# spool-labs/clay

Hardware: AMD Instinct MI355X
Metric: device-resident encode GiB/s at (k=10,m=4,d=13); % of HBM roofline (higher is better)
Workload: dtype u8; 1 GPU; (k=10,m=4,d=13) encode, one 1 GiB stripe per GPU; stripe_input_bytes=1073741824, padded_stripe_bytes=1073745920, chunk_bytes=107374592, sub_chunk_bytes=419432, alpha=256, parallelism=stripe-per-gpu x1

## Files before the change

bench_tools/stream_probe.hip:

```cpp
#include <hip/hip_runtime.h>

#include <algorithm>
#include <cstdlib>
#include <cstdio>
#include <vector>

#include "../clay_amd/csrc/stream_encode.hpp"

using namespace clay::bs;

template <int L, int PROBE>
static float run(BsArgs a, int reps) {
    using Kn = StreamEnc<10, L>;
    (void)hipFuncSetAttribute(reinterpret_cast<const void *>(&k_stream_encode<10, L, PROBE>),
                              hipFuncAttributeMaxDynamicSharedMemorySize, Kn::LDS_BYTES);
    hipEvent_t e0, e1;
    (void)hipEventCreate(&e0);
    (void)hipEventCreate(&e1);
    std::vector<float> t;
    for (int r = 0; r < reps; r++) {
        (void)hipEventRecord(e0);
        k_stream_encode<10, L, PROBE><<<dim3(a.nslots * 8), dim3(Kn::BLOCK), Kn::LDS_BYTES>>>(a);
        (void)hipEventRecord(e1);
        (void)hipEventSynchronize(e1);
        float ms;
        (void)hipEventElapsedTime(&ms, e0, e1);
        if (r >= 3) t.push_back(ms);
    }
    std::sort(t.begin(), t.end());
    return t[t.size() / 2];
}

template <int L, int PROBE, int MAP = 0>
static float run_b2b(BsArgs a, int n, int warm = 50) {
    using Kn = StreamEnc<10, L>;
    (void)hipFuncSetAttribute(reinterpret_cast<const void *>(&k_stream_encode<10, L, PROBE, MAP>),
                              hipFuncAttributeMaxDynamicSharedMemorySize, Kn::LDS_BYTES);
    hipEvent_t e0, e1;
    (void)hipEventCreate(&e0);
    (void)hipEventCreate(&e1);
    for (int i = 0; i < warm; i++)
        k_stream_encode<10, L, PROBE, MAP><<<dim3(a.nslots * 8), dim3(Kn::BLOCK), Kn::LDS_BYTES>>>(a);
    (void)hipEventRecord(e0);
    for (int i = 0; i < n; i++)
        k_stream_encode<10, L, PROBE, MAP><<<dim3(a.nslots * 8), dim3(Kn::BLOCK), Kn::LDS_BYTES>>>(a);
    (void)hipEventRecord(e1);
    (void)hipEventSynchronize(e1);
    float ms;
    (void)hipEventElapsedTime(&ms, e0, e1);
    const hipError_t err = hipGetLastError();
    if (err != hipSuccess) {
        printf("HIP error (probe %d): %s\n", PROBE, hipGetErrorString(err));
        exit(3);
    }
    return ms / float(n);
}

template <int TP, int MAP = 0>
static void timing_report(BsArgs a, int n) {
    using Kn = StreamEnc<10, 4>;
    const int grid = int(a.nslots) * 8;
    const size_t rec = size_t(grid) * 12 * 24;
    uint64_t *tb;
    (void)hipMalloc(&tb, rec * 8);
    (void)hipMemset(tb, 0, rec * 8);
    a.par[4] = reinterpret_cast<uint8_t *>(tb);
    const float ms_plain = run_b2b<4, 0, MAP>(a, n);
    const float ms_tm = run_b2b<4, TP, MAP>(a, n);
    std::vector<uint64_t> h(rec);
    (void)hipMemcpy(h.data(), tb, rec * 8, hipMemcpyDeviceToHost);
    printf("b2b ms: plain %.4f  timing-probe %.4f (s_memtime counts per XCD; cycles below are per tile)\n", ms_plain, ms_tm);
    printf("wave  role     total   bar/vm y0   y1    y2 | math/bar y0   y1    y2 | issue y0  y1    y2 | end g0  g1    g2    g3\n");
    for (int w = 0; w < 12; w++) {
        double v[3][3] = {}, ge[4] = {}, tot = 0;
        int cnt = 0;
        for (int b = 0; b < grid; b++) {
            const uint64_t *p = &h[(size_t(b) * 12 + w) * 24];
            const double nt = double(p[16]);
            if (nt == 0) continue;
            cnt++;
            for (int i = 0; i < 3; i++)
                for (int j = 0; j < 3; j++) v[i][j] += double(p[i * 3 + j]) / nt;
            for (int g = 0; g < 4; g++) ge[g] += double(p[9 + g]) / nt;
            tot += double(p[15] - p[13]) / nt;
        }
        const double G = cnt ? cnt : 1;
        printf("%4d  %-7s %7.0f  %6.0f %6.0f %6.0f | %6.0f %6.0f %6.0f | %6.0f %6.0f %6.0f | %5.0f %5.0f %5.0f %5.0f\n", w,
               w < 8 ? "compute" : "loader", tot / G, v[0][0] / G, v[0][1] / G, v[0][2] / G, v[1][0] / G, v[1][1] / G,
               v[1][2] / G, v[2][0] / G, v[2][1] / G, v[2][2] / G, ge[0] / G, ge[1] / G, ge[2] / G, ge[3] / G);
    }
    fflush(stdout);
    (void)hipFree(tb);
    (void)Kn::BLOCK;
}

int main(int argc, char **argv) {
    const uint32_t sc = argc > 1 ? uint32_t(atoi(argv[1])) : 419432;
    const bool quick = argc > 2;
    const size_t chunk = size_t(sc) * 256;
    uint8_t *data, *par;
    if (hipMalloc(&data, 10 * chunk) != hipSuccess || hipMalloc(&par, 4 * chunk) != hipSuccess) return 1;
    {
        std::vector<uint8_t> h(10 * chunk);
        uint64_t x = 0x9E3779B97F4A7C15ull;
        for (auto &b : h) { x ^= x << 13; x ^= x >> 7; x ^= x << 17; b = uint8_t(x >> 24); }
        (void)hipMemcpy(data, h.data(), h.size(), hipMemcpyHostToDevice);
    }
    BsArgs a{};
    for (int i = 0; i < 10; i++) a.data[i] = data + i * chunk;
    for (int x = 0; x < 4; x++) a.par[x] = par + x * chunk;
    a.sc = sc;
    const uint32_t ralign = argc > 3 ? uint32_t(atoi(argv[3])) : 32u;
    a.tiles_per_xcd = uint32_t(((sc + 7) / 8 + ralign - 1) / ralign * ralign);
    a.nslots = 32;
    const double bytes = 14.0 * chunk;
    auto rep = [&](const char *n, float ms) {
        printf("%-34s %8.4f ms  %7.1f GB/s (algorithmic)\n", n, ms, bytes / (ms * 1e-3) / 1e9);
        fflush(stdout);
    };
    (void)hipFuncSetAttribute(reinterpret_cast<const void *>(&k_stream_encode<10, 2, 0>),
                              hipFuncAttributeMaxDynamicSharedMemorySize, StreamEnc<10, 2>::LDS_BYTES);
    for (int i = 0; i < 300; i++) k_stream_encode<10, 2, 0><<<dim3(a.nslots * 8), dim3(StreamEnc<10, 2>::BLOCK), StreamEnc<10, 2>::LDS_BYTES>>>(a);
    {
        const hipError_t e = hipDeviceSynchronize();
        const hipError_t e2 = hipGetLastError();
        if (e != hipSuccess || e2 != hipSuccess) {
            printf("HIP error after warm-up: %s / %s\n", hipGetErrorString(e), hipGetErrorString(e2));
            return 3;
        }
    }
    if (argc > 2 && argv[2][0] == 't') {
        printf("sc %u segment timing\n", sc);
        timing_report<4096>(a, 200);
        printf("---- deferred end of group (PROBE 8192)\n");
        timing_report<4096 | 8192>(a, 200);
        return 0;
    }
    if (argc > 2 && argv[2][0] == 'd') {
        printf("sc %u deferred end-of-group A/B, back-to-back\n", sc);
        for (int rr = 0; rr < 3; rr++) {
            rep("b2b full", run_b2b<4, 0>(a, 200));
            rep("b2b full, end of group after the next barrier", run_b2b<4, 8192>(a, 200));
            rep("b2b memory only", run_b2b<4, 1>(a, 200));
            rep("b2b memory only, deferred", run_b2b<4, 8193>(a, 200));
            rep("b2b full, no sched barrier between nodes", run_b2b<4, 16384>(a, 200));
            rep("b2b full, sched barrier every 2 nodes", run_b2b<4, 32768>(a, 200));
            rep("b2b full, deferred + every 2 nodes", run_b2b<4, 32768 | 8192>(a, 200));
        }
        return 0;
    }
    if (argc > 2 && argv[2][0] == 'p') {
        printf("sc %u balanced priority A/B, back-to-back\n", sc);
        for (int rr = 0; rr < 3; rr++) {
            rep("b2b full", run_b2b<4, 0>(a, 200));
            rep("b2b full, balanced priority", run_b2b<4, 131072>(a, 200));
            rep("b2b math + stores (no DMA)", run_b2b<4, 2>(a, 200));
            rep("b2b math + stores (no DMA), balanced priority", run_b2b<4, 2 | 131072>(a, 200));
        }
        timing_report<4096 | 131072>(a, 200);
        return 0;
    }
    if (argc > 2 && argv[2][0] == 'v') {
        printf("sc %u variants, back-to-back (200 launches after 50 untimed)\n", sc);
        for (int rr = 0; rr < 3; rr++) {
            rep("b2b full", run_b2b<4, 0>(a, 200));
            rep("b2b memory only (DMA + stores, no math)", run_b2b<4, 1>(a, 200));
            rep("b2b reads only", run_b2b<4, 5>(a, 200));
            rep("b2b stores only", run_b2b<4, 3>(a, 200));
            rep("b2b live reads + math (no stores)", run_b2b<4, 262144>(a, 200));
            rep("b2b live math only (no DMA, no stores)", run_b2b<4, 262146>(a, 200));
            rep("b2b math + stores (no DMA)", run_b2b<4, 2>(a, 200));
            rep("b2b math + stores, no DMA, no barriers", run_b2b<4, 2 | 65536>(a, 200));
            rep("b2b live math only, no barriers", run_b2b<4, 262146 | 65536>(a, 200));
        }
        return 0;
    }
    if (argc > 2 && argv[2][0] == 'n') {
        printf("sc %u lane map A/B, back-to-back (200 launches after 50 untimed)\n", sc);
        if (argv[2][1] == 't') {
            timing_report<4096, 0>(a, 200);
            printf("---- map 3\n");
            timing_report<4096, 3>(a, 200);
            return 0;
        }
        const size_t pbytes = 4 * chunk;
        std::vector<uint8_t> ref(pbytes), got(pbytes);
        auto snap = [&](std::vector<uint8_t> &v) {
            (void)hipDeviceSynchronize();
            (void)hipMemcpy(v.data(), par, pbytes, hipMemcpyDeviceToHost);
        };
        (void)hipMemset(par, 0, pbytes);
        run_b2b<4, 0, 0>(a, 1, 0);
        snap(ref);
        auto check = [&](const char *name) {
            snap(got);
            printf("  bytes %s == map 0: %s\n", name, ref == got ? "yes" : "NO");
            (void)hipMemset(par, 0, pbytes);
        };
        run_b2b<4, 0, 1>(a, 1, 0); check("map 1");
        run_b2b<4, 0, 3>(a, 1, 0); check("map 3");
        run_b2b<4, 0, 4>(a, 1, 0); check("map 4");
        run_b2b<4, 0, 5>(a, 1, 0); check("map 5");
        run_b2b<4, 0, 6>(a, 1, 0); check("map 6");
        run_b2b<4, 0, 7>(a, 1, 0); check("map 7");
        run_b2b<4, 0, 8>(a, 1, 0); check("map 8");
        run_b2b<4, 0, 9>(a, 1, 0); check("map 9");
        if (argv[2][1] == '8') {
            for (int rr = 0; rr < 3; rr++) {
                rep("b2b full, map 0 (round 5)", run_b2b<4, 0, 0>(a, 200));
                rep("b2b full, map 8", run_b2b<4, 0, 8>(a, 200));
                rep("b2b full, map 9 (map 8 without red skip)", run_b2b<4, 0, 9>(a, 200));
                rep("b2b full, map 8, waves 4-7 prio 1", run_b2b<4, 16, 8>(a, 200));
                rep("b2b full, map 8, no sched barriers", run_b2b<4, 16384, 8>(a, 200));
                rep("b2b full, map 8, sched barrier / 2 nodes", run_b2b<4, 32768, 8>(a, 200));
                rep("b2b memory only, map 8", run_b2b<4, 1, 8>(a, 200));
                rep("b2b live math only, map 8", run_b2b<4, 262146, 8>(a, 200));
                rep("b2b live reads + math, map 8", run_b2b<4, 262144, 8>(a, 200));
                rep("b2b math + stores, map 8", run_b2b<4, 2, 8>(a, 200));
            }
            timing_report<4096, 8>(a, 200);
            return 0;
        }
        for (int rr = 0; rr < 3; rr++) {
            rep("b2b full, map 0 (round 5)", run_b2b<4, 0, 0>(a, 200));
            rep("b2b memory only, map 0", run_b2b<4, 1, 0>(a, 200));
            rep("b2b full, map 1 (k 2,3,4 pair 16)", run_b2b<4, 0, 1>(a, 200));
            rep("b2b memory only, map 1", run_b2b<4, 1, 1>(a, 200));
            rep("b2b full, map 3 (map 1, permlane pair 32)", run_b2b<4, 0, 3>(a, 200));
            rep("b2b full, map 4 (k 3,2,4 pair 32)", run_b2b<4, 0, 4>(a, 200));
            rep("b2b memory only, map 4", run_b2b<4, 1, 4>(a, 200));
            rep("b2b full, map 5 (k 4,3,2 pair 64)", run_b2b<4, 0, 5>(a, 200));
            rep("b2b memory only, map 5", run_b2b<4, 1, 5>(a, 200));
            rep("b2b full, map 6 (k 5,4,3 pair 128)", run_b2b<4, 0, 6>(a, 200));
            rep("b2b memory only, map 6", run_b2b<4, 1, 6>(a, 200));
            rep("b2b full, map 7 (k 2,5,4 pair 16)", run_b2b<4, 0, 7>(a, 200));
            rep("b2b memory only, map 7", run_b2b<4, 1, 7>(a, 200));
            rep("b2b full, map 8 (k 4,5,3 pair 64)", run_b2b<4, 0, 8>(a, 200));
            rep("b2b memory only, map 8", run_b2b<4, 1, 8>(a, 200));
            rep("b2b live math only, map 1", run_b2b<4, 262146, 1>(a, 200));
        }
        return 0;
    }
    if (argc > 2 && argv[2][0] == 'w') {
        rep("full", run_b2b<4, 0>(a, 10, 2));
        rep("memory only", run_b2b<4, 1>(a, 10, 2));
        rep("reads only", run_b2b<4, 5>(a, 10, 2));
        rep("stores only", run_b2b<4, 3>(a, 10, 2));
        rep("live reads + math", run_b2b<4, 262144>(a, 10, 2));
        rep("live math only", run_b2b<4, 262146>(a, 10, 2));
        rep("math + stores", run_b2b<4, 2>(a, 10, 2));
        return 0;
    }
    if (argc > 2 && argv[2][0] == 'f') {
        unsigned int *flag;
        (void)hipMalloc(&flag, 4);
        (void)hipMemset(flag, 0, 4);
        a.par[5] = reinterpret_cast<uint8_t *>(flag);
        printf("sc %u no-barrier timing probe (PROBE 4096|65536|2) with bounds checks (524288)\n", sc);
        timing_report<4096 | 65536 | 2 | 524288>(a, 50);
        unsigned int h = 0;
        (void)hipMemcpy(&h, flag, 4, hipMemcpyDeviceToHost);
        printf("bounds flags 0x%x (bits 0-3 parity store of node X, 4-7 ragged store, 8 compute record, 9 loader record)\n", h);
        return 0;
    }
    if (argc > 2 && argv[2][0] == 'a') {
        printf("sc %u (row start mod 128 varies: %s), XCD region %u (alignment %u)\n", sc,
               sc % 128 ? "yes" : "no, rows 128-aligned", a.tiles_per_xcd, ralign);
        for (int rr = 0; rr < 2; rr++) {
            rep("b2b full", run_b2b<4, 0>(a, 200));
            rep("b2b memory only (DMA + stores)", run_b2b<4, 1>(a, 200));
            rep("b2b stores only", run_b2b<4, 3>(a, 200));
            rep("b2b reads only", run_b2b<4, 5>(a, 200));
        }
        return 0;
    }
    if (argc > 2 && argv[2][0] == 'l') {
        printf("sc %u back-to-back loader sweep\n", sc);
        for (int rr = 0; rr < 3; rr++) {
            rep("b2b L4 full", run_b2b<4, 0>(a, 200));
            rep("b2b L2 full", run_b2b<2, 0>(a, 200));
            rep("b2b L1 full", run_b2b<1, 0>(a, 200));
            rep("b2b L4 full, loaders prio 0", run_b2b<4, 8>(a, 200));
        }
        return 0;
    }
    if (argc > 2 && argv[2][0] == 'b') {
        printf("sc %u back-to-back (200 launches after 50 untimed)\n", sc);
        for (int rr = 0; rr < 3; rr++) {
            rep("b2b L4 full (CSE)", run_b2b<4, 0>(a, 200));
            rep("b2b L4 full, no CSE", run_b2b<4, 1024>(a, 200));
            rep("b2b L4 memory only", run_b2b<4, 1>(a, 200));
            rep("b2b L4 math + stores (CSE)", run_b2b<4, 2>(a, 200));
        }
        return 0;
    }
    if (argc > 2 && argv[2][0] == 'm') {
        printf("sc %u tile map (XCD-blocked vs chip round robin), back-to-back\n", sc);
        for (int rr = 0; rr < 3; rr++) {
            rep("b2b full, XCD-blocked", run_b2b<4, 0>(a, 200));
            rep("b2b full, chip RR", run_b2b<4, 2048>(a, 200));
            rep("b2b memory only, XCD-blocked", run_b2b<4, 1>(a, 200));
            rep("b2b memory only, chip RR", run_b2b<4, 2049>(a, 200));
            rep("b2b stores only, XCD-blocked", run_b2b<4, 3>(a, 200));
            rep("b2b stores only, chip RR", run_b2b<4, 2051>(a, 200));
            rep("b2b reads only, XCD-blocked", run_b2b<4, 5>(a, 200));
            rep("b2b reads only, chip RR", run_b2b<4, 2053>(a, 200));
        }
        return 0;
    }
    if (argc > 2 && argv[2][0] == 'x') {
        printf("sc %u cse folds\n", sc);
        for (int rr = 0; rr < 3; rr++) {
            rep("L4 full, row-by-row folds", run<4, 1024>(a, 15));
            rep("L4 full (CSE folds)", run<4, 0>(a, 15));
            rep("L0 full, row-by-row folds", run<0, 1024>(a, 15));
            rep("L0 full (CSE folds)", run<0, 0>(a, 15));
            rep("L4 math + stores, row-by-row folds", run<4, 1026>(a, 15));
            rep("L4 math + stores (CSE folds)", run<4, 2>(a, 15));
        }
        return 0;
    }
    if (argc > 2 && argv[2][0] == 'c') {
        printf("sc %u cache policies\n", sc);
        for (int rr = 0; rr < 2; rr++) {
            rep("L4 full", run<4, 0>(a, 15));
            rep("L4 full, nt loads", run<4, 64>(a, 15));
            rep("L4 full, nt stores", run<4, 256>(a, 15));
            rep("L4 full, nt loads + stores", run<4, 320>(a, 15));
            rep("L4 full, sc1 loads", run<4, 128>(a, 15));
            rep("L4 full, sc1 stores", run<4, 512>(a, 15));
            rep("L4 memory only", run<4, 1>(a, 15));
            rep("L4 memory only, nt loads", run<4, 65>(a, 15));
            rep("L4 memory only, nt stores", run<4, 257>(a, 15));
            rep("L4 memory only, nt both", run<4, 321>(a, 15));
            rep("L4 reads, nt", run<4, 69>(a, 15));
            rep("L4 stores only, nt", run<4, 259>(a, 15));
        }
        return 0;
    }
    if (quick) {
        printf("sc %u\n", sc);
        for (int rr = 0; rr < 2; rr++) {
            rep("L4 full", run<4, 0>(a, 15));
            rep("L4 no math (memory only)", run<4, 1>(a, 15));
            rep("L4 reads", run<4, 5>(a, 15));
            rep("L4 stores only", run<4, 3>(a, 15));
            rep("L4 memory only, rotated stores", run<4, 33>(a, 15));
            rep("L4 stores only, rotated", run<4, 35>(a, 15));
        }
        return 0;
    }
    for (int rr = 0; rr < 2; rr++) {
        rep("L0 full", run<0, 0>(a, 15));
        rep("L1 full", run<1, 0>(a, 15));
        rep("L2 full", run<2, 0>(a, 15));
        rep("L4 full loaders prio 0", run<4, 8>(a, 15));
        rep("L4 full waves 4-7 prio 1", run<4, 16>(a, 15));
        rep("L2 full waves 4-7 prio 1", run<2, 16>(a, 15));
        rep("L4 full", run<4, 0>(a, 15));
        rep("L0 no math (memory only)", run<0, 1>(a, 15));
        rep("L4 no math (memory only)", run<4, 1>(a, 15));
        rep("L0 reads", run<0, 5>(a, 15));
        rep("L4 reads", run<4, 5>(a, 15));
        rep("L4 no DMA (math + stores)", run<4, 2>(a, 15));
        rep("L4 stores only", run<4, 3>(a, 15));
    }
    return 0;
}
```

clay_amd/csrc/stream_encode.hpp:

```cpp
#pragma once

#include "encode_math.hpp"

namespace clay {
namespace bs {

__device__ __forceinline__ const uint8_t *uniform_ptr(const uint8_t *p) {
    const uint64_t v = reinterpret_cast<uint64_t>(p);
    const uint32_t lo = __builtin_amdgcn_readfirstlane(uint32_t(v)), hi = __builtin_amdgcn_readfirstlane(uint32_t(v >> 32));
    return reinterpret_cast<const uint8_t *>((uint64_t(hi) << 32) | lo);
}

struct StreamTile {
    uint32_t b0, vend;
};

struct StreamMap {
    uint32_t x0, x1, nfull, p0, p1, w;
    __device__ StreamMap(uint32_t sc, uint32_t region, uint32_t ns, uint32_t xcd, uint32_t slot, uint32_t W = 256u) {
        w = W;
        x0 = xcd * region;
        x1 = x0 + region < sc ? x0 + region : sc;
        nfull = p0 = p1 = 0;
        if (x0 >= x1) return;
        const uint32_t len = x1 - x0, round = ns * W;
        nfull = len / round;
        const uint32_t left = len - nfull * round;
        const uint32_t wp = ((left + ns - 1) / ns + 31u) & ~31u;
        const uint32_t q0 = x0 + nfull * round + slot * wp;
        if (left && q0 < x1) {
            p0 = q0;
            p1 = q0 + wp < x1 ? q0 + wp : x1;
        }
    }
    __device__ int ntile() const { return int(nfull) + (p0 < p1 ? 1 : 0); }
    __device__ StreamTile tile(int k, uint32_t slot, uint32_t ns) const {
        if (uint32_t(k) < nfull) {
            const uint32_t b0 = x0 + (uint32_t(k) * ns + slot) * w;
            return {b0, b0 + w};
        }
        return {p0, p1};
    }
};

struct ChipMap {
    uint32_t b, G, nfull, pend, sc;
    __device__ ChipMap(uint32_t sc_, uint32_t b_, uint32_t G_) : b(b_), G(G_), nfull(sc_ / 256u), sc(sc_) {
        pend = (sc_ % 256u) && (nfull % G_) == b_ ? 1u : 0u;
    }
    __device__ int ntile() const { return int((nfull > b ? (nfull - b + G - 1) / G : 0u) + pend); }
    __device__ StreamTile tile(int k, uint32_t, uint32_t) const {
        const uint32_t t = b + uint32_t(k) * G;
        if (t < nfull) return {t * 256u, t * 256u + 256u};
        return {nfull * 256u, sc};
    }
};

template <int KD, int LOADERS, int CPL = 0, int CPS = 0, bool CSE = true, bool SINK = false, bool CHECK = false,
          int MAP = 0>
struct StreamEnc {
    using K6 = EncMath<KD>;
    using S = typename K6::S;
    static constexpr int Q = 4, T = 4, W = 256, CWAVES = 8;
    static constexpr int BLOCK = 64 * (CWAVES + LOADERS);
    static constexpr int NODE_BYTES = 64 * W;
    static constexpr int REGION = Q * NODE_BYTES;
    static constexpr int LDS_BYTES = KD * NODE_BYTES;
    static constexpr int STEPS = 12;
    static constexpr int DMA_WAVES = LOADERS ? LOADERS : CWAVES;
    static constexpr int BPL = 16 / DMA_WAVES;
    static_assert(LOADERS == 0 || LOADERS == 1 || LOADERS == 2 || LOADERS == 4, "loader waves");
    static_assert(KD >= 9 && KD <= 10 && LDS_BYTES <= 160 * 1024, "one 16 KiB buffer per data node");

    static constexpr int nreal(int y) {
        int n = 0;
        for (int x = 0; x < Q; x++) n += (y * Q + x < KD);
        return n;
    }
    static constexpr int ninstr(int y) { return nreal(y) * BPL; }
    static constexpr int nstores(int g) { return 2 * (1 + 2 * g); }
    static constexpr int dshift(int y) { return 2 * (T - 2 - y); }

    __host__ __device__ static constexpr uint32_t sw(uint32_t r) { return ((r >> 1) & 1u) * 8u; }
    struct MapSpec {
        int kb0, kb1, kb2, wb, swb;
        bool light_old, pswap, redskip;
    };
    static constexpr MapSpec spec() {
        switch (MAP) {
            case 1: return {2, 3, 4, 5, 3, false, false, true};
            case 2: return {2, 3, 4, 5, 3, true, false, true};
            case 3: return {2, 3, 4, 5, 3, false, true, true};
            case 4: return {3, 2, 4, 5, 3, false, false, true};
            case 5: return {4, 3, 2, 5, 3, false, false, true};
            case 6: return {5, 4, 3, 2, 5, false, false, true};
            case 7: return {2, 5, 4, 3, 5, false, false, true};
            case 8: return {4, 5, 3, 2, 5, false, false, true};
            case 9: return {4, 5, 3, 2, 5, false, false, false};
            default: return {0, 1, 2, 3, 1, false, false, false};
        }
    }
    static constexpr MapSpec MS = spec();
    static constexpr bool PSWAP = MS.pswap;
    static constexpr uint32_t PAIR = MAP == 0 ? 4u : (4u << (PSWAP ? MS.kb1 : MS.kb0));
    __device__ static int colmap(int w, int k) {
        if constexpr (MAP == 0) return 8 * w + k;
        const int hi = MS.light_old ? (((w >> 2) & 1) ^ 1) : ((w >> 2) & 1);
        return (w & 1) | (hi << 1) | ((k & 1) << MS.kb0) | (((k >> 1) & 1) << MS.kb1) | (((k >> 2) & 1) << MS.kb2) |
               (((w >> 1) & 1) << MS.wb);
    }
    __host__ __device__ static constexpr uint32_t swn(uint32_t x, uint32_t r) {
        return MAP == 0 ? sw(r) : ((((r >> MS.swb) & 1u) ^ ((x >> 1) & 1u))) * 8u;
    }
    static constexpr bool sw_in_digit(int y) { return MS.swb == dshift(y) || MS.swb == dshift(y) + 1; }
    static constexpr int comp_swap(int y, int x) { return sw_in_digit(y) ? ((x >> (MS.swb - dshift(y))) & 1) : 0; }

    struct Loader {
        uint32_t off[2][BPL];
        uint32_t rl;
        uint32_t slot;
        int li;
    };
    __device__ static uint32_t k16_of(const Loader &L, int j, uint32_t b) {
        const uint32_t r = uint32_t(L.li * BPL + j) * 4u + L.rl;
        return (L.slot ^ swn(b * 2u, r)) * 16u;
    }
    __device__ static void loader_init(Loader &L, uint32_t sc, int li, int lane) {
        L.li = li;
        L.rl = uint32_t(lane) >> 4;
        L.slot = uint32_t(lane) & 15u;
#pragma unroll
        for (int j = 0; j < BPL; j++) {
            const uint32_t r = uint32_t(li * BPL + j) * 4u + L.rl;
            L.off[0][j] = r * 4u * sc + k16_of(L, j, 0u);
            L.off[1][j] = r * 4u * sc + k16_of(L, j, 1u);
        }
    }
    template <int Y>
    __device__ static void issue(const BsArgs &a, const Loader &L, uint32_t lds0, StreamTile t, int g) {
        const uint32_t sc = uint32_t(a.sc);
        const bool full = t.vend >= t.b0 + uint32_t(W);
        sfor<Q>([&](auto xc) BS_INL {
            constexpr int x = decltype(xc)::value;
            constexpr int node = Y * Q + x;
            if constexpr (node < KD) {
                constexpr uint32_t b = (uint32_t(x) >> 1) & 1u;
                const uint32_t dst = lds0 + uint32_t(node * NODE_BYTES) + uint32_t(L.li * BPL) * 1024u;
                if (full) {
                    const uint8_t *base = uniform_ptr(a.data[node] + (uint64_t(g) * sc + t.b0));
#pragma unroll
                    for (int j = 0; j < BPL; j++) dma16p<CPL>(dst + uint32_t(j) * 1024u, base, L.off[b][j]);
                } else {
                    const uint8_t *base = uniform_ptr(a.data[node] + uint64_t(g) * sc);
#pragma unroll
                    for (int j = 0; j < BPL; j++) {
                        const uint32_t k16 = k16_of(L, j, b);
                        uint32_t pos = t.b0 + k16;
                        if (pos + 16u > t.vend) pos = t.vend - 16u;
                        dma16p<CPL>(dst + uint32_t(j) * 1024u, base, L.off[b][j] - k16 + pos);
                    }
                }
            }
        });
    }
    __device__ static void issue_any(int y, const BsArgs &a, const Loader &L, uint32_t lds0, StreamTile t, int g) {
        if (y == 0) issue<0>(a, L, lds0, t, g);
        else if (y == 1) issue<1>(a, L, lds0, t, g);
        else issue<2>(a, L, lds0, t, g);
    }
    template <int Y>
    __device__ static void patch(const BsArgs &a, const Loader &L, uint8_t *smem, StreamTile t, int g, int lane) {
        const uint32_t sc = uint32_t(a.sc);
        sfor<Q>([&](auto xc) BS_INL {
            constexpr int x = decltype(xc)::value;
            constexpr int node = Y * Q + x;
            if constexpr (node < KD) {
#pragma unroll
                for (int j = 0; j < BPL; j++) {
                    const uint32_t pos = t.b0 + k16_of(L, j, (uint32_t(x) >> 1) & 1u);
                    if (!(pos < t.vend && pos + 16u > t.vend)) continue;
                    const int blk = L.li * BPL + j;
                    const uint32_t layer = (uint32_t(blk) * 4u + L.rl) * 4u + uint32_t(g);
                    const uint2 gv = *reinterpret_cast<const uint2 *>(a.data[node] + uint64_t(layer) * sc + pos);
                    *reinterpret_cast<uint4 *>(smem + node * NODE_BYTES + blk * 1024 + lane * 16) =
                        make_uint4(gv.x, gv.y, 0u, 0u);
                }
            }
        });
    }
    __device__ static void patch_any(int y, const BsArgs &a, const Loader &L, uint8_t *smem, StreamTile t, int g,
                                     int lane) {
        if (y == 0) patch<0>(a, L, smem, t, g, lane);
        else if (y == 1) patch<1>(a, L, smem, t, g, lane);
        else patch<2>(a, L, smem, t, g, lane);
    }

    struct LaneS {
        uint32_t own[2], cb[3][2];
        int cy[3];
    };
    __device__ static LaneS lane_consts(int c, int part) {
        LaneS L;
        if constexpr (MAP != 0) {
            const uint32_t uc = uint32_t(c), up = uint32_t(part);
            L.own[0] = uc * 256u + ((up ^ (((uc >> MS.swb) & 1u) * 8u)) * 16u);
            L.own[1] = L.own[0] ^ 128u;
#pragma unroll
            for (int y = 0; y < 3; y++) {
                const int sh = dshift(y);
                L.cy[y] = (c >> sh) & 3;
                const uint32_t cy = uint32_t(L.cy[y]);
                const uint32_t row0 = (uc & ~(3u << sh)) * 256u + cy * uint32_t(NODE_BYTES);
                const uint32_t rb = sw_in_digit(y) ? 0u : ((uc >> MS.swb) & 1u);
                L.cb[y][0] = row0 + ((up ^ ((rb ^ ((cy >> 1) & 1u)) * 8u)) * 16u);
                L.cb[y][1] = L.cb[y][0] ^ 128u;
            }
            return L;
        }
        const uint32_t pk = (uint32_t(part) ^ sw(uint32_t(c))) * 16u;
        L.own[0] = uint32_t(c) * 256u + pk;
        L.own[1] = L.own[0] ^ 128u;
#pragma unroll
        for (int y = 0; y < 3; y++) {
            const int sh = dshift(y);
            L.cy[y] = (c >> sh) & 3;
            const uint32_t row0 = uint32_t(c & ~(3 << sh)) * 256u + uint32_t(L.cy[y]) * uint32_t(NODE_BYTES);
            if (y < 2) {
                L.cb[y][0] = row0 + pk;
                L.cb[y][1] = L.cb[y][0] ^ 128u;
            } else {
                L.cb[y][0] = L.cb[y][1] = row0 + uint32_t(part) * 16u;
            }
        }
        return L;
    }
    __device__ static void read32(const uint8_t *p0, const uint8_t *p1, uint32_t (&d)[8]) {
        const uint4 v0 = *reinterpret_cast<const uint4 *>(p0), v1 = *reinterpret_cast<const uint4 *>(p1);
        d[0] = v0.x; d[1] = v0.y; d[2] = v0.z; d[3] = v0.w;
        d[4] = v1.x; d[5] = v1.y; d[6] = v1.z; d[7] = v1.w;
    }
    template <int Y, int X>
    __device__ static void load_x(const uint8_t *slot, const LaneS &L, uint32_t (&o)[8], uint32_t (&cv)[8]) {
        if constexpr (MAP != 0) {
            constexpr int bx = (X >> 1) & 1;
            if constexpr (Y * Q + X < KD) {
                read32(slot + X * NODE_BYTES + L.own[bx], slot + X * NODE_BYTES + L.own[bx ^ 1], o);
            } else {
#pragma unroll
                for (int w = 0; w < 8; w++) o[w] = 0;
            }
            if ((Y * Q + L.cy[Y]) < KD && (Y != 2 || !MS.redskip || X != L.cy[Y])) {
                constexpr uint32_t step = uint32_t(256) << dshift(Y);
                constexpr int hb = comp_swap(Y, X);
                read32(slot + L.cb[Y][hb] + X * step, slot + L.cb[Y][hb ^ 1] + X * step, cv);
            } else {
#pragma unroll
                for (int w = 0; w < 8; w++) cv[w] = 0;
            }
            return;
        }
        if constexpr (Y * Q + X < KD) {
            read32(slot + X * NODE_BYTES + L.own[0], slot + X * NODE_BYTES + L.own[1], o);
        } else {
#pragma unroll
            for (int w = 0; w < 8; w++) o[w] = 0;
        }
        if ((Y * Q + L.cy[Y]) < KD) {
            constexpr uint32_t step = uint32_t(256) << dshift(Y);
            if constexpr (Y < 2) {
                read32(slot + L.cb[Y][0] + X * step, slot + L.cb[Y][1] + X * step, cv);
            } else {
                constexpr uint32_t s0 = sw(uint32_t(X)) * 16u;
                read32(slot + L.cb[Y][0] + (X * step + s0), slot + L.cb[Y][0] + (X * step + (s0 ^ 128u)), cv);
            }
        } else {
#pragma unroll
            for (int w = 0; w < 8; w++) cv[w] = 0;
        }
    }
    template <int Y, int X>
    __device__ static void prt_x(const uint32_t (&o)[8], const uint32_t (&cv)[8], const LaneS &L, uint32_t (&u)[8]) {
        const int cy = L.cy[Y];
        if constexpr (MAP != 0 && Y == 2 && MS.redskip) {
            if (X == cy) {
#pragma unroll
                for (int w = 0; w < 8; w++) u[w] = o[w];
                return;
            }
        }
        const bool creal = (Y * Q + cy) < KD;
        const uint32_t keep = (creal && X != cy) ? 0xffffffffu : 0u;
        const uint32_t ks = keep & 0xfefefefeu, kr = keep & 0x1d1d1d1du;
#pragma unroll
        for (int w = 0; w < 8; w++) u[w] = xor_xtime4_masked(o[w], cv[w], ks, kr);
    }
    template <int Y, int SBN = 1, bool BAL = false>
    __device__ __forceinline__ static void section(const uint8_t *slot, const LaneS &L, uint32_t (&acc)[Q * 8]) {
        uint32_t o[2][8], cv[2][8];
        if constexpr (BAL) __builtin_amdgcn_s_setprio(1);
        load_x<Y, 0>(slot, L, o[0], cv[0]);
        sfor<Q>([&](auto xc) BS_INL {
            constexpr int x = decltype(xc)::value;
            if constexpr (BAL && x == 2) __builtin_amdgcn_s_setprio(0);
            if constexpr (x + 1 < Q) load_x<Y, x + 1>(slot, L, o[(x + 1) & 1], cv[(x + 1) & 1]);
            uint32_t u[8];
            prt_x<Y, x>(o[x & 1], cv[x & 1], L, u);
            if constexpr (CSE) K6::template fold_x_cse<Y, x>(u, acc);
            else K6::template fold_x<Y, x>(u, acc);
            if constexpr (SBN > 0 && (x + 1) % SBN == 0) __builtin_amdgcn_sched_barrier(0);
        });
    }

    template <int D2, int SBN = 1>
    __device__ __forceinline__ static void section2_u(const uint8_t *slot, const LaneS &L, uint32_t (&acc)[Q * 8]) {
        static_assert(MAP != 0, "wave-uniform digit 2");
        constexpr int Y = 2;
        auto load = [&](auto xc, uint32_t (&o)[8], uint32_t (&cv)[8]) BS_INL {
            constexpr int x = decltype(xc)::value;
            constexpr bool own_real = Y * Q + x < KD;
            constexpr bool comp_real = x != D2 && Y * Q + D2 < KD;
            constexpr int bx = (x >> 1) & 1;
            if constexpr (own_real) read32(slot + x * NODE_BYTES + L.own[bx], slot + x * NODE_BYTES + L.own[bx ^ 1], o);
            constexpr int hb = comp_swap(Y, x);
            if constexpr (comp_real) read32(slot + L.cb[Y][hb] + x * 256, slot + L.cb[Y][hb ^ 1] + x * 256, cv);
        };
        uint32_t o[2][8], cv[2][8];
        load(std::integral_constant<int, 0>{}, o[0], cv[0]);
        sfor<Q>([&](auto xc) BS_INL {
            constexpr int x = decltype(xc)::value;
            constexpr bool own_real = Y * Q + x < KD;
            constexpr bool comp_real = x != D2 && Y * Q + D2 < KD;
            if constexpr (x + 1 < Q) load(std::integral_constant<int, x + 1>{}, o[(x + 1) & 1], cv[(x + 1) & 1]);
            if constexpr (own_real || comp_real) {
                uint32_t u[8];
#pragma unroll
                for (int w = 0; w < 8; w++) {
                    if constexpr (own_real && comp_real) u[w] = xor_xtime4_masked(o[x & 1][w], cv[x & 1][w], 0xfefefefeu, 0x1d1d1d1du);
                    else if constexpr (comp_real) u[w] = xor_xtime4_masked(0u, cv[x & 1][w], 0xfefefefeu, 0x1d1d1d1du);
                    else u[w] = o[x & 1][w];
                }
                if constexpr (CSE) K6::template fold_x_cse<Y, x>(u, acc);
                else K6::template fold_x<Y, x>(u, acc);
                if constexpr (SBN > 0) __builtin_amdgcn_sched_barrier(0);
            }
        });
        asm volatile("; section2_u end %0" ::"n"(D2));
    }

    __device__ __forceinline__ static void pair_halves(const uint32_t (&cv)[8], uint32_t (&lo)[4], uint32_t (&hi)[4]) {
        if constexpr (PSWAP) {
#pragma unroll
            for (int i = 0; i < 4; i++) {
                const auto r = __builtin_amdgcn_permlane16_swap(cv[i], cv[4 + i], false, false);
                lo[i] = r[0];
                hi[i] = r[1];
            }
        } else {
            const bool odd = (threadIdx.x >> 3) & 1u;
#pragma unroll
            for (int i = 0; i < 4; i++) {
                const uint32_t send = odd ? cv[i] : cv[4 + i];
                const uint32_t r = uint32_t(__builtin_amdgcn_update_dpp(0, int(send), 0x128, 0xf, 0xf, false));
                lo[i] = odd ? r : cv[i];
                hi[i] = odd ? cv[4 + i] : r;
            }
        }
    }
    template <int X>
    __device__ __forceinline__ static void put(const BsArgs &a, uint32_t (&cv)[8], uint32_t z, StreamTile t, uint32_t prel,
                               bool ragged, uint32_t &sink) {
        transpose8(cv);
        if (SINK && !ragged) {
            uint32_t lo[4], hi[4];
            pair_halves(cv, lo, hi);
            sink ^= xor3(xor3(lo[0], lo[1], lo[2]), xor3(lo[3], hi[0], hi[1]), hi[2] ^ hi[3]);
            sink += X;
            return;
        }
        if (SINK) {
            sink ^= xor3(xor3(cv[0], cv[1], cv[2]), xor3(cv[3], cv[4], cv[5]), cv[6] ^ cv[7]);
            return;
        }
        (void)sink;
        if (!ragged) {
            const bool odd = PSWAP ? ((threadIdx.x >> 4) & 1u) : ((threadIdx.x >> 3) & 1u);
            uint32_t lo[4], hi[4];
            pair_halves(cv, lo, hi);
            uint32_t off = (z - (odd ? PAIR : 0u)) * uint32_t(a.sc);
            asm volatile("" : "+v"(off));
            off += t.b0 + prel + (odd ? 128u : 0u);
            const uint8_t *base = uniform_ptr(a.par[X]);
            if constexpr (CHECK) {
                const uint64_t lim = uint64_t(a.sc) * 256u;
                if (uint64_t(off) + 16u > lim || uint64_t(off) + PAIR * a.sc + 16u > lim) {
                    atomicOr(reinterpret_cast<unsigned int *>(a.par[5]), 1u << X);
                    return;
                }
            }
            st16sp<CPS>(base, off, lo[0], lo[1], lo[2], lo[3]);
            st16sp<CPS>(base, off + PAIR * uint32_t(a.sc), hi[0], hi[1], hi[2], hi[3]);
        } else {
            uint8_t *p = a.par[X] + uint64_t(z) * a.sc + t.b0 + prel;
#pragma unroll
            for (int h = 0; h < 2; h++) {
                const uint32_t pos = t.b0 + prel + 128u * uint32_t(h);
                const uint32_t nv = pos >= t.vend ? 0u : (t.vend - pos >= 16u ? 16u : t.vend - pos);
                if constexpr (CHECK) {
                    if (nv && (z >= 256u || pos + nv > a.sc)) {
                        atomicOr(reinterpret_cast<unsigned int *>(a.par[5]), 16u << X);
                        continue;
                    }
                }
                if (nv == 16u)
                    *reinterpret_cast<uint4 *>(p + 128 * h) = make_uint4(cv[4 * h], cv[4 * h + 1], cv[4 * h + 2], cv[4 * h + 3]);
                else if (nv >= 8u)
                    *reinterpret_cast<uint2 *>(p + 128 * h) = make_uint2(cv[4 * h], cv[4 * h + 1]);
            }
        }
    }
    template <int G>
    __device__ __forceinline__ static void end_group(const BsArgs &a, const uint32_t (&acc)[Q * 8], typename K6::Hold &H, int c,
                                     StreamTile t, uint32_t prel, bool ragged, uint32_t &sink) {
        const uint32_t zg = uint32_t(c * 4 + G);
        uint32_t cv[8];
#pragma unroll
        for (int w = 0; w < 8; w++) cv[w] = acc[G * 8 + w];
        put<G>(a, cv, zg, t, prel, ragged, sink);
        auto pair = [&](const uint32_t *uh_at_g, const uint32_t *ug_at_h, auto hc) BS_INL {
            constexpr int h = decltype(hc)::value;
            const uint32_t zh = uint32_t(c * 4 + h);
            uint32_t c12[16];
            if constexpr (CSE) {
                K6::pft_pair(uh_at_g, ug_at_h, c12);
            } else {
                uint32_t c1[8], c2[8];
                K6::pft(uh_at_g, ug_at_h, c1);
                K6::pft(ug_at_h, uh_at_g, c2);
#pragma unroll
                for (int w = 0; w < 8; w++) {
                    c12[w] = c1[w];
                    c12[8 + w] = c2[w];
                }
            }
            uint32_t c1[8], c2[8];
#pragma unroll
            for (int w = 0; w < 8; w++) {
                c1[w] = c12[w];
                c2[w] = c12[8 + w];
            }
            put<h>(a, c1, zg, t, prel, ragged, sink);
            put<G>(a, c2, zh, t, prel, ragged, sink);
        };
        auto keep = [&](int ri, int p) BS_INL {
#pragma unroll
            for (int w = 0; w < 8; w++) H.r[ri][w] = acc[p * 8 + w];
        };
        if constexpr (G == 0) {
            keep(0, 1);
            keep(1, 2);
            keep(2, 3);
        } else if constexpr (G == 1) {
            pair(acc + 0, H.r[0], std::integral_constant<int, 0>{});
            keep(0, 2);
            keep(3, 3);
        } else if constexpr (G == 2) {
            pair(acc + 0, H.r[1], std::integral_constant<int, 0>{});
            pair(acc + 8, H.r[0], std::integral_constant<int, 1>{});
            keep(1, 3);
        } else {
            pair(acc + 0, H.r[2], std::integral_constant<int, 0>{});
            pair(acc + 8, H.r[3], std::integral_constant<int, 1>{});
            pair(acc + 16, H.r[1], std::integral_constant<int, 2>{});
        }
    }
};

struct TimeAcc {
    uint64_t v[3][3] = {{0, 0, 0}, {0, 0, 0}, {0, 0, 0}}, gend[4] = {0, 0, 0, 0};
    uint64_t t_start = 0, t_first = 0, t_end = 0;
    __device__ __forceinline__ void add(int kind, int y, uint64_t &t0) {
        const uint64_t t1 = __builtin_amdgcn_s_memtime();
        const uint64_t d = t1 - t0;
        t0 = t1;
        if (y == 0) v[kind][0] += d;
        else if (y == 1) v[kind][1] += d;
        else v[kind][2] += d;
    }
    __device__ __forceinline__ void addg(int g, uint64_t &t0) {
        const uint64_t t1 = __builtin_amdgcn_s_memtime();
        const uint64_t d = t1 - t0;
        t0 = t1;
        if (g == 0) gend[0] += d;
        else if (g == 1) gend[1] += d;
        else if (g == 2) gend[2] += d;
        else gend[3] += d;
    }
    __device__ void put(uint64_t *p, int ntile) const {
        for (int i = 0; i < 3; i++)
            for (int j = 0; j < 3; j++) p[i * 3 + j] = v[i][j];
        for (int g = 0; g < 4; g++) p[9 + g] = gend[g];
        p[13] = t_start;
        p[14] = t_first;
        p[15] = t_end;
        p[16] = uint64_t(ntile);
    }
};

constexpr int kStreamEncMap = 8;

template <int KD, int LOADERS, int PROBE = 0, int MAP = 0>
__global__ __launch_bounds__((StreamEnc<KD, LOADERS>::BLOCK)) void k_stream_encode(BsArgs a) {
    using Kn = StreamEnc<KD, LOADERS, (PROBE >> 6) & 3, (PROBE >> 8) & 3, ((PROBE >> 10) & 1) == 0, (PROBE & 262144) != 0,
                         (PROBE & 524288) != 0, MAP>;
    uint32_t sink = 0;
    constexpr bool TM = (PROBE & 4096) != 0;
    using K6 = typename Kn::K6;
    extern __shared__ __attribute__((aligned(16))) uint8_t smem[];
    const int wave = __builtin_amdgcn_readfirstlane(threadIdx.x >> 6), lane = threadIdx.x & 63;
    const uint32_t xcd = blockIdx.x & 7u, slot = blockIdx.x >> 3, ns = a.nslots;
    const auto tm = [&] {
        if constexpr ((PROBE & 2048) != 0) return ChipMap(uint32_t(a.sc), blockIdx.x, gridDim.x);
        else return StreamMap(uint32_t(a.sc), a.tiles_per_xcd, ns, xcd, slot);
    }();
    const int ntile = tm.ntile();
    if (ntile == 0) return;
    const int nsteps = ntile * Kn::STEPS;
    if (LOADERS > 0 && wave >= Kn::CWAVES) {
        if constexpr (!(PROBE & 8)) __builtin_amdgcn_s_setprio(3);
        typename Kn::Loader L;
        Kn::loader_init(L, uint32_t(a.sc), wave - Kn::CWAVES, lane);
        const uint32_t lds0 = lds_addr_of(smem);
        TimeAcc T;
        T.t_start = TM ? __builtin_amdgcn_s_memtime() : 0;
        if constexpr (!(PROBE & 2))
            for (int s = 0; s < 3 && s < nsteps; s++) Kn::issue_any(s % 3, a, L, lds0, tm.tile(0, slot, ns), s / 3);
        uint64_t t0 = TM ? __builtin_amdgcn_s_memtime() : 0;
        if constexpr (TM) T.t_first = t0;
        for (int s = 0; s < nsteps; s++) {
            const int k = s / Kn::STEPS, r = s % Kn::STEPS, g = r / 3, y = r % 3;
            const StreamTile t = tm.tile(k, slot, ns);
            int after = 0;
            if (s == 0) {
                after = (nsteps > 1 ? Kn::ninstr(1) : 0) + (nsteps > 2 ? Kn::ninstr(2) : 0);
            } else if (s + 1 < nsteps) {
                after = Kn::ninstr((y + 1) % 3);
            }
            const bool straddle = t.vend < t.b0 + uint32_t(Kn::W) && ((t.vend - t.b0) & 15u);
            if (PROBE & 2) {
            } else if (straddle) {
                wait_vm_n<0>();
                Kn::patch_any(y, a, L, smem, t, g, lane);
            } else {
                wait_vm_rt(after);
            }
            if constexpr (TM) T.add(0, y, t0);
            if constexpr (!(PROBE & 65536)) lds_barrier();
            if constexpr (TM) T.add(1, y, t0);
            const int s2 = s + 2;
            if (!(PROBE & 2) && s >= 1 && s2 < nsteps) {
                const int k2 = s2 / Kn::STEPS, r2 = s2 % Kn::STEPS;
                Kn::issue_any(r2 % 3, a, L, lds0, tm.tile(k2, slot, ns), r2 / 3);
            }
            if constexpr (TM) T.add(2, y, t0);
        }
        if constexpr (TM) {
            T.t_end = __builtin_amdgcn_s_memtime();
            const uint32_t rec = blockIdx.x * 12u + uint32_t(wave);
            if ((PROBE & 524288) != 0 && (rec >= gridDim.x * 12u || wave >= 12)) {
                if (lane == 0) atomicOr(reinterpret_cast<unsigned int *>(a.par[5]), 512u);
            } else if (lane == 0) {
                T.put(reinterpret_cast<uint64_t *>(a.par[4]) + rec * 24u, ntile);
            }
        }
        return;
    }
    if constexpr ((PROBE & 16) != 0) {
        if (wave >= 4) __builtin_amdgcn_s_setprio(1);
    }
    const int c = Kn::colmap(wave, (int(threadIdx.x) >> 3) & 7), part = int(threadIdx.x) & 7;
    constexpr bool SEC2U = (PROBE & 1048576) != 0;
    const uint32_t prel = uint32_t(part) * 16u;
    uint32_t acc[Kn::Q * 8];
    typename K6::Hold H;
    const typename Kn::LaneS LC = Kn::lane_consts(c, part);
    typename Kn::Loader LD;
    const uint32_t lds0 = lds_addr_of(smem);
    if constexpr (LOADERS == 0) {
        Kn::loader_init(LD, uint32_t(a.sc), wave, lane);
        if constexpr (!(PROBE & 2))
            for (int s = 0; s < 3 && s < nsteps; s++) Kn::issue_any(s % 3, a, LD, lds0, tm.tile(0, slot, ns), s / 3);
    }
    int st1 = 0, st2 = 0;
    constexpr bool DEFER = (PROBE & 8192) != 0 && LOADERS > 0;
    int pend = -1;
    StreamTile pt{0, 0};
    auto end_any = [&](int ge, StreamTile t) BS_INL {
        const bool ragged = t.vend < t.b0 + uint32_t(Kn::W);
        int cc = c;
        asm volatile("" : "+v"(cc));
        if (ge == 0) Kn::template end_group<0>(a, acc, H, cc, t, prel, ragged, sink);
        else if (ge == 1) Kn::template end_group<1>(a, acc, H, cc, t, prel, ragged, sink);
        else if (ge == 2) Kn::template end_group<2>(a, acc, H, cc, t, prel, ragged, sink);
        else Kn::template end_group<3>(a, acc, H, cc, t, prel, ragged, sink);
    };
    TimeAcc T;
    T.t_start = TM ? __builtin_amdgcn_s_memtime() : 0;
    uint64_t t0 = TM ? __builtin_amdgcn_s_memtime() : 0;
    if constexpr (TM) T.t_first = t0;
    for (int s = 0; s < nsteps; s++) {
        const int k = s / Kn::STEPS, r = s % Kn::STEPS, g = r / 3, y = r % 3;
        if constexpr (LOADERS == 0 && !(PROBE & 2)) {
            const StreamTile t = tm.tile(k, slot, ns);
            int after;
            if (s == 0) after = (nsteps > 1 ? Kn::ninstr(1) : 0) + (nsteps > 2 ? Kn::ninstr(2) : 0);
            else if (s == 1) after = (nsteps > 2 ? Kn::ninstr(2) : 0) + st1;
            else after = st2 + (s + 1 < nsteps ? Kn::ninstr((y + 1) % 3) : 0) + st1;
            if (t.vend < t.b0 + uint32_t(Kn::W) && ((t.vend - t.b0) & 15u)) {
                wait_vm_n<0>();
                Kn::patch_any(y, a, LD, smem, t, g, lane);
            } else {
                wait_vm_rt(after);
            }
        }
        if constexpr (!(PROBE & 65536)) lds_barrier();
        if constexpr (TM) T.add(0, y, t0);
        if constexpr (DEFER) {
            if (pend >= 0) {
                end_any(pend, pt);
                if constexpr (TM) T.addg(pend, t0);
                pend = -1;
            }
        }
        if constexpr (LOADERS == 0 && !(PROBE & 2)) {
            const int s2 = s + 2;
            if (s >= 1 && s2 < nsteps) {
                const int k2 = s2 / Kn::STEPS, r2 = s2 % Kn::STEPS;
                Kn::issue_any(r2 % 3, a, LD, lds0, tm.tile(k2, slot, ns), r2 / 3);
            }
        }
        typename Kn::LaneS L = LC;
        asm volatile("" : "+v"(L.own[0]), "+v"(L.own[1]), "+v"(L.cb[0][0]), "+v"(L.cb[0][1]));
        asm volatile("" : "+v"(L.cb[1][0]), "+v"(L.cb[1][1]), "+v"(L.cb[2][0]));
        if constexpr (MAP != 0) {
            asm volatile("" : "+v"(L.cb[2][1]));
            asm volatile("" : "+v"(L.cy[0]), "+v"(L.cy[1]));
            L.cy[2] = __builtin_amdgcn_readfirstlane(L.cy[2]);
        } else {
            asm volatile("" : "+v"(L.cy[0]), "+v"(L.cy[1]), "+v"(L.cy[2]));
        }
        if constexpr ((PROBE & 1) != 0) {
            if (s == 0)
#pragma unroll
                for (int w = 0; w < Kn::Q * 8; w++) acc[w] = (threadIdx.x * 0x9E3779B9u) ^ uint32_t(w) ^ L.own[0];
        } else {
            constexpr int SBN = (PROBE & 16384) ? 0 : (PROBE & 32768) ? 2 : 1;
            constexpr bool BAL = (PROBE & 131072) != 0;
            if (y == 0) Kn::template section<0, SBN, BAL>(smem, L, acc);
            else if (y == 1) Kn::template section<1, SBN, BAL>(smem + Kn::REGION, L, acc);
            else if constexpr (MAP != 0) {
                const int d2 = L.cy[2];
                if constexpr (SEC2U) {
                    if (d2 == 0) Kn::template section2_u<0, SBN>(smem + 2 * Kn::REGION, L, acc);
                    else if (d2 == 1) Kn::template section2_u<1, SBN>(smem + 2 * Kn::REGION, L, acc);
                    else Kn::template section2_u<2, SBN>(smem + 2 * Kn::REGION, L, acc);
                } else {
                    if (d2 >= 2) Kn::template section2_u<2, SBN>(smem + 2 * Kn::REGION, L, acc);
                    else Kn::template section<2, SBN, BAL>(smem + 2 * Kn::REGION, L, acc);
                }
            } else Kn::template section<2, SBN, BAL>(smem + 2 * Kn::REGION, L, acc);
        }
        if constexpr (TM) T.add(1, y, t0);
        if (y == 2 && !(PROBE & 4)) {
            const StreamTile t = tm.tile(k, slot, ns);
            const bool ragged = t.vend < t.b0 + uint32_t(Kn::W);
            const int ge = (PROBE & 32) ? ((g + int(slot)) & 3) : g;
            if constexpr (DEFER) {
                pend = ge;
                pt = t;
            } else {
                end_any(ge, t);
            }
            st2 = st1;
            st1 = ragged ? 0 : Kn::nstores(ge);
        } else {
            st2 = st1;
            st1 = 0;
        }
        if constexpr (TM) T.addg(g, t0);
    }
    if constexpr (DEFER) {
        if (pend >= 0) end_any(pend, pt);
    }
    if constexpr ((PROBE & 262144) != 0) {
        if (sink == uint32_t(a.sdata) + 0x9E3779B9u) a.par[0][threadIdx.x] = uint8_t(sink);
    }
    if constexpr (TM) {
        T.t_end = __builtin_amdgcn_s_memtime();
        const uint32_t rec = blockIdx.x * 12u + uint32_t(wave);
        if ((PROBE & 524288) != 0 && (rec >= gridDim.x * 12u || wave >= 12)) {
            if (lane == 0) atomicOr(reinterpret_cast<unsigned int *>(a.par[5]), 256u);
        } else if (lane == 0) {
            T.put(reinterpret_cast<uint64_t *>(a.par[4]) + rec * 24u, ntile);
        }
    }
}

}
}
```

Measured before the change: 2941 GiB/s.

## Balance stream tile rounds across slots and predicate ragged tile loads with exec masks

Replaces the default per-XCD tile map with a BalancedMap that spreads each XCD region evenly over all rounds in 16-byte pieces. This removes the old layout of full 256-column rounds followed by a narrow, unevenly sized tail. Tiles narrower than 256 but 16-aligned are no longer treated as ragged. Loads for them use exec-masked global_load_lds (when the LPRED probe bit is set), and stores skip lanes past the tile end. The aim is to cut tail imbalance between blocks, at the cost of more partial tiles and extra per-store bounds checks.

After: 3017 GiB/s, median of 6. 2.6% higher.

```diff
diff --git a/bench_tools/stream_probe.hip b/bench_tools/stream_probe.hip
--- a/bench_tools/stream_probe.hip
+++ b/bench_tools/stream_probe.hip
@@ -241,6 +241,37 @@
         }
         return 0;
     }
+    if (argc > 2 && argv[2][0] == 'r') {
+        constexpr int M = kStreamEncMap, OLD = 2097152;
+        printf("sc %u tile map A/B (balanced rounds vs full rounds + narrow tail), back-to-back (200 launches after 50 untimed)\n", sc);
+        const size_t pbytes = 4 * chunk;
+        std::vector<uint8_t> ref(pbytes), got(pbytes);
+        (void)hipMemset(par, 0, pbytes);
+        run_b2b<4, OLD, M>(a, 1, 0);
+        (void)hipDeviceSynchronize();
+        (void)hipMemcpy(ref.data(), par, pbytes, hipMemcpyDeviceToHost);
+        (void)hipMemset(par, 0xA5, pbytes);
+        run_b2b<4, 0, M>(a, 1, 0);
+        (void)hipDeviceSynchronize();
+        (void)hipMemcpy(got.data(), par, pbytes, hipMemcpyDeviceToHost);
+        printf("  bytes new == old: %s\n", ref == got ? "yes" : "NO");
+        (void)hipMemset(par, 0x5A, pbytes);
+        run_b2b<4, 4194304, M>(a, 1, 0);
+        (void)hipDeviceSynchronize();
+        (void)hipMemcpy(got.data(), par, pbytes, hipMemcpyDeviceToHost);
+        printf("  bytes new, masked loads (PROBE 4194304) == old: %s\n", ref == got ? "yes" : "NO");
+        for (int rr = 0; rr < 3; rr++) {
+            rep("b2b full, old map", run_b2b<4, OLD, M>(a, 200));
+            rep("b2b full, balanced map", run_b2b<4, 0, M>(a, 200));
+            rep("b2b memory only, old map", run_b2b<4, OLD | 1, M>(a, 200));
+            rep("b2b memory only, balanced map", run_b2b<4, 1, M>(a, 200));
+            rep("b2b live math only, old map", run_b2b<4, OLD | 262146, M>(a, 200));
+            rep("b2b live math only, balanced map", run_b2b<4, 262146, M>(a, 200));
+            rep("b2b full, balanced map, masked loads", run_b2b<4, 4194304, M>(a, 200));
+            rep("b2b memory only, balanced, masked loads", run_b2b<4, 4194304 | 1, M>(a, 200));
+        }
+        return 0;
+    }
     if (argc > 2 && argv[2][0] == 'w') {
         rep("full", run_b2b<4, 0>(a, 10, 2));
         rep("memory only", run_b2b<4, 1>(a, 10, 2));
diff --git a/clay_amd/csrc/stream_encode.hpp b/clay_amd/csrc/stream_encode.hpp
--- a/clay_amd/csrc/stream_encode.hpp
+++ b/clay_amd/csrc/stream_encode.hpp
@@ -1,6 +1,7 @@
 #pragma once
 
 #include "encode_math.hpp"
+#include "stream_tile_map.hpp"
 
 namespace clay {
 namespace bs {
@@ -11,9 +12,16 @@
     return reinterpret_cast<const uint8_t *>((uint64_t(hi) << 32) | lo);
 }
 
-struct StreamTile {
-    uint32_t b0, vend;
-};
+__device__ __forceinline__ void dma16_masked(uint32_t lds_addr, const uint8_t *sbase, uint32_t voff, uint64_t mask) {
+    unsigned keep;
+    uint64_t ex;
+    asm volatile(
+        "s_mov_b32 %0, m0\n\ts_mov_b32 m0, %2\n\ts_mov_b64 %1, exec\n\ts_mov_b64 exec, %5\n\t"
+        "global_load_lds_dwordx4 %3, %4\n\ts_mov_b64 exec, %1\n\ts_mov_b32 m0, %0"
+        : "=&s"(keep), "=&s"(ex)
+        : "s"(lds_addr), "v"(voff), "s"(sbase), "s"(mask)
+        : "memory");
+}
 
 struct StreamMap {
     uint32_t x0, x1, nfull, p0, p1, w;
@@ -57,7 +65,7 @@
 };
 
 template <int KD, int LOADERS, int CPL = 0, int CPS = 0, bool CSE = true, bool SINK = false, bool CHECK = false,
-          int MAP = 0>
+          int MAP = 0, bool LPRED = false>
 struct StreamEnc {
     using K6 = EncMath<KD>;
     using S = typename K6::S;
@@ -150,6 +158,13 @@
                     const uint8_t *base = uniform_ptr(a.data[node] + (uint64_t(g) * sc + t.b0));
 #pragma unroll
                     for (int j = 0; j < BPL; j++) dma16p<CPL>(dst + uint32_t(j) * 1024u, base, L.off[b][j]);
+                } else if (LPRED && ((t.vend - t.b0) & 15u) == 0) {
+                    const uint8_t *base = uniform_ptr(a.data[node] + (uint64_t(g) * sc + t.b0));
+#pragma unroll
+                    for (int j = 0; j < BPL; j++) {
+                        const uint64_t mask = __builtin_amdgcn_ballot_w64(k16_of(L, j, b) + 16u <= t.vend - t.b0);
+                        dma16_masked(dst + uint32_t(j) * 1024u, base, L.off[b][j], mask);
+                    }
                 } else {
                     const uint8_t *base = uniform_ptr(a.data[node] + uint64_t(g) * sc);
 #pragma unroll
@@ -388,8 +403,15 @@
             pair_halves(cv, lo, hi);
             uint32_t off = (z - (odd ? PAIR : 0u)) * uint32_t(a.sc);
             asm volatile("" : "+v"(off));
-            off += t.b0 + prel + (odd ? 128u : 0u);
+            uint32_t pos = prel + (odd ? 128u : 0u);
+            if constexpr (!PSWAP) {
+                uint32_t l = threadIdx.x;
+                asm volatile("" : "+v"(l));
+                pos = (l & 15u) << 4;
+            }
+            off += t.b0 + pos;
             const uint8_t *base = uniform_ptr(a.par[X]);
+            if (pos + 16u > t.vend - t.b0) return;
             if constexpr (CHECK) {
                 const uint64_t lim = uint64_t(a.sc) * 256u;
                 if (uint64_t(off) + 16u > lim || uint64_t(off) + PAIR * a.sc + 16u > lim) {
@@ -511,17 +533,22 @@
 template <int KD, int LOADERS, int PROBE = 0, int MAP = 0>
 __global__ __launch_bounds__((StreamEnc<KD, LOADERS>::BLOCK)) void k_stream_encode(BsArgs a) {
     using Kn = StreamEnc<KD, LOADERS, (PROBE >> 6) & 3, (PROBE >> 8) & 3, ((PROBE >> 10) & 1) == 0, (PROBE & 262144) != 0,
-                         (PROBE & 524288) != 0, MAP>;
+                         (PROBE & 524288) != 0, MAP, (PROBE & 4194304) != 0>;
     uint32_t sink = 0;
     constexpr bool TM = (PROBE & 4096) != 0;
     using K6 = typename Kn::K6;
     extern __shared__ __attribute__((aligned(16))) uint8_t smem[];
     const int wave = __builtin_amdgcn_readfirstlane(threadIdx.x >> 6), lane = threadIdx.x & 63;
     const uint32_t xcd = blockIdx.x & 7u, slot = blockIdx.x >> 3, ns = a.nslots;
+    constexpr bool OLDMAP = (PROBE & (2048 | 2097152)) != 0;
     const auto tm = [&] {
         if constexpr ((PROBE & 2048) != 0) return ChipMap(uint32_t(a.sc), blockIdx.x, gridDim.x);
-        else return StreamMap(uint32_t(a.sc), a.tiles_per_xcd, ns, xcd, slot);
+        else if constexpr (OLDMAP) return StreamMap(uint32_t(a.sc), a.tiles_per_xcd, ns, xcd, slot);
+        else return BalancedMap(uint32_t(a.sc), a.tiles_per_xcd, ns, xcd, slot);
     }();
+    const auto is_ragged = [](StreamTile t) BS_INL {
+        return OLDMAP ? t.vend < t.b0 + uint32_t(Kn::W) : ((t.vend - t.b0) & 15u) != 0;
+    };
     const int ntile = tm.ntile();
     if (ntile == 0) return;
     const int nsteps = ntile * Kn::STEPS;
@@ -595,7 +622,7 @@
     int pend = -1;
     StreamTile pt{0, 0};
     auto end_any = [&](int ge, StreamTile t) BS_INL {
-        const bool ragged = t.vend < t.b0 + uint32_t(Kn::W);
+        const bool ragged = is_ragged(t);
         int cc = c;
         asm volatile("" : "+v"(cc));
         if (ge == 0) Kn::template end_group<0>(a, acc, H, cc, t, prel, ragged, sink);
@@ -672,7 +699,7 @@
         if constexpr (TM) T.add(1, y, t0);
         if (y == 2 && !(PROBE & 4)) {
             const StreamTile t = tm.tile(k, slot, ns);
-            const bool ragged = t.vend < t.b0 + uint32_t(Kn::W);
+            const bool ragged = is_ragged(t);
             const int ge = (PROBE & 32) ? ((g + int(slot)) & 3) : g;
             if constexpr (DEFER) {
                 pend = ge;
diff --git a/clay_amd/csrc/stream_tile_map.hpp b/clay_amd/csrc/stream_tile_map.hpp
--- /dev/null
+++ b/clay_amd/csrc/stream_tile_map.hpp
@@ -0,0 +1,46 @@
+#pragma once
+
+#include <cstdint>
+
+#if defined(__HIPCC__) || defined(__CUDACC__)
+#define CLAY_TILE_MAP_HD __host__ __device__
+#else
+#define CLAY_TILE_MAP_HD
+#endif
+
+namespace clay {
+namespace bs {
+
+struct StreamTile {
+    uint32_t b0, vend;
+};
+
+struct BalancedMap {
+    uint32_t x0, x1, nrounds, q, rem, nt;
+    CLAY_TILE_MAP_HD BalancedMap(uint32_t sc, uint32_t region, uint32_t ns, uint32_t xcd, uint32_t slot) {
+        x0 = xcd * region;
+        x1 = x0 + region < sc ? x0 + region : sc;
+        nrounds = q = rem = nt = 0;
+        if (x0 >= x1) return;
+        const uint32_t len = x1 - x0;
+        nrounds = (len + ns * 256u - 1u) / (ns * 256u);
+        const uint32_t pieces = (len + ns * 16u - 1u) / (ns * 16u);
+        q = pieces / nrounds;
+        rem = pieces % nrounds;
+        nt = start(nrounds - 1u, slot, ns) < x1 ? nrounds : nrounds - 1u;
+    }
+    CLAY_TILE_MAP_HD uint32_t width(uint32_t r) const { return (q + (r < rem ? 1u : 0u)) * 16u; }
+    CLAY_TILE_MAP_HD uint32_t start(uint32_t r, uint32_t slot, uint32_t ns) const {
+        const uint32_t before = r * q + (r < rem ? r : rem);
+        return x0 + (ns * before + slot * (q + (r < rem ? 1u : 0u))) * 16u;
+    }
+    CLAY_TILE_MAP_HD int rounds() const { return int(nrounds); }
+    CLAY_TILE_MAP_HD int ntile() const { return int(nt); }
+    CLAY_TILE_MAP_HD StreamTile tile(int k, uint32_t slot, uint32_t ns) const {
+        const uint32_t b0 = start(uint32_t(k), slot, ns), e = b0 + width(uint32_t(k));
+        return {b0, e < x1 ? e : x1};
+    }
+};
+
+}
+}
```
